# LaurenYTaylor/jsrl-CORL

Hardware: AMD Instinct MI355X
Metric: IQL gradient-steps/sec at batch=256 (D4RL obs/act dims) (higher is better)
Workload: dtype f32; 1 GPU; IQL step on synthetic buffer (obs=17, act=6, 1000000 rows), batch=256 per GPU; global_batch=256, parallelism=single, prepare_rehearsal_steps=1111

## Files before the change

include/iqlhip.h:

```cpp
#ifndef IQLHIP_H
#define IQLHIP_H

#include <stdint.h>

#ifdef __cplusplus
extern "C" {
#endif

#define IQLHIP_VERSION 400
#define IQLHIP_HIDDEN 256
#define IQLHIP_MAX_INPUT 128
#define IQLHIP_MAX_ACTION 32
#define IQLHIP_MAX_WORLD 8
#define IQLHIP_GRAPH_STEPS 64
#define IQLHIP_N_SCORE 8
#define IQLHIP_N_STATS 16

enum {
  IQLHIP_OK = 0,
  IQLHIP_EINVAL = -1,
  IQLHIP_EHIP = -2,
  IQLHIP_ENOTBOUND = -3,
  IQLHIP_EUNSUPPORTED = -4,
  IQLHIP_EINDEX = -5,
  IQLHIP_EEXCHANGE = -6
};

enum { IQLHIP_NET_V = 0, IQLHIP_NET_Q1 = 1, IQLHIP_NET_Q2 = 2, IQLHIP_NET_PI = 3 };
enum { IQLHIP_POLICY_GAUSSIAN = 0, IQLHIP_POLICY_DETERMINISTIC = 1 };

typedef struct {
  int32_t state_dim;
  int32_t action_dim;
  int32_t hidden_dim;
  int32_t n_hidden;
  int32_t policy;
  int32_t max_batch;
} iqlhip_dims;

typedef struct {
  int64_t seg_begin, seg_end;
  int64_t w0, b0, w1, b1, w2, b2, log_std;
  int32_t k_in;
  int32_t d_out;
} iqlhip_net_layout;

typedef struct {
  iqlhip_net_layout net[4];
  int64_t n_params;
  int64_t n_target;
  int64_t target_src;
} iqlhip_layout;

int iqlhip_arena_layout(const iqlhip_dims* dims, iqlhip_layout* out);

typedef struct {
  float iql_tau;
  float beta;
  float discount;
  float tau;
  float one_minus_tau;
  float exp_adv_max;
  float log_std_min, log_std_max;
} iqlhip_hyper;

typedef struct {
  float step_size[3];
  float bc2_sqrt[3];
  float beta2;
  float one_minus_beta1;
  float one_minus_beta2;
  float eps;
  float grad_scale;
  float inv_batch;
} iqlhip_step_scalars;

typedef struct {
  const float* s_dev; const float* a_dev; const float* r_dev; const float* ns_dev; const float* d_dev;
  int64_t ld_s, ld_a, ld_r, ld_ns, ld_d;
  const int64_t* idx_dev;
  int32_t rows;
} iqlhip_batch;

typedef struct iqlhip_ctx iqlhip_ctx;

int iqlhip_version(void);
const char* iqlhip_last_error(void);
// ... 300 lines not shown
```

jsrl-corl_amd/csrc/iqlhip.hip:

```cpp
#include "iqlhip_kernels.h"
#include "iqlhip_lb_kernels.h"
#include "iqlhip_owned.h"

#include <dlfcn.h>

#include <time.h>

#include <algorithm>
#include <cstdarg>
#include <cstdio>
#include <cstdlib>
#include <cstring>
#include <memory>
#include <string>
#include <type_traits>
#include <vector>

#define GRAPH_STEPS IQLHIP_GRAPH_STEPS
static const int kChunkSizes[] = {GRAPH_STEPS, 16, 4, 2, 1};

static thread_local std::string g_err;

static int fail(int code, const char* fmt, ...) {
  char buf[512];
// ... 278 lines not shown
    iqlhip_net_layout& nl = out->net[n];
    nl.k_in = (n == IQLHIP_NET_Q1 || n == IQLHIP_NET_Q2) ? S + A : S;
    nl.d_out = (n == IQLHIP_NET_PI) ? A : 1;
    nl.seg_begin = off;
    nl.w1 = off; off += (int64_t)Hd * Hd;
    nl.w0 = off; off += (int64_t)Hd * nl.k_in;
    nl.b0 = off; off += Hd;
    nl.b1 = off; off += Hd;
    nl.w2 = off; off += (int64_t)nl.d_out * Hd;
    nl.b2 = off; off += up(nl.d_out, 4);
    if (n == IQLHIP_NET_PI && d->policy == IQLHIP_POLICY_GAUSSIAN) { nl.log_std = off; off += up(A, 4); }
    else nl.log_std = -1;
    off = up(off, 64);
    nl.seg_end = off;
  }
  out->n_params = off;
  out->target_src = out->net[IQLHIP_NET_Q1].seg_begin;
  out->n_target = out->net[IQLHIP_NET_Q2].seg_end - out->net[IQLHIP_NET_Q1].seg_begin;
  return IQLHIP_OK;
}

extern "C" int64_t iqlhip_row_stride(int32_t S, int32_t A) { return up(2 * (int64_t)S + A + 2, 4); }

static int xld_host(int k0) { int k0p = (k0 + 3) & ~3; return ((k0p + 29) / 32) * 32 + 2; }

extern "C" int iqlhip_destroy(iqlhip_ctx* c);
extern "C" int iqlhip_xch_shutdown(iqlhip_ctx* c);

static int create_impl(iqlhip_ctx* c, const iqlhip_dims* dims, const iqlhip_hyper* hyper, int device) {
  c->dims = *dims;
  c->hyper = *hyper;
  c->device = device;
  iqlhip_arena_layout(dims, &c->L);
  const int MB = dims->max_batch, A = dims->action_dim;
  c->n_chunk_max = (MB + CHUNK_ROWS - 1) / CHUNK_ROWS;
  c->n_rt_max = (MB + RT_ROWS - 1) / RT_ROWS;
  c->sc.max_batch = MB;
  Owned& own = c->own;
  auto dalloc = [&](float** p, size_t nfloat) { return own.dev(p, nfloat * sizeof(float), 0); };
  HIPCHK(dalloc(&c->sc.h0, (size_t)4 * MB * HID));
  HIPCHK(dalloc(&c->sc.h1, (size_t)4 * MB * HID));
  HIPCHK(dalloc(&c->sc.heads, (size_t)MB * HEAD_LD + (size_t)NSPLIT * MB * A));
  c->row_ld = iqlhip_row_stride(dims->state_dim, A);
  HIPCHK(dalloc(&c->xb, (size_t)MB * c->row_ld));
  HIPCHK(dalloc(&c->xb2, (size_t)MB * c->row_ld));
  HIPCHK(own.pin(&c->losses_host, 4 * sizeof(float)));
  HIPCHK(own.pin(&c->on_row_pin, (size_t)c->row_ld * sizeof(float)));
  HIPCHK(own.pin(&c->on_idx_pin, (size_t)MB * sizeof(long long)));
  HIPCHK(own.pin(&c->on_loss_pin, 4 * sizeof(float)));
  HIPCHK(own.pin(&c->done_pin, 8 * sizeof(unsigned long long), true));
  HIPCHK(own.pin(&c->on_act_pin, (size_t)(IQLHIP_MAX_INPUT + IQLHIP_MAX_ACTION) * sizeof(float)));
  c->act_cap = std::max(MB, IQLHIP_ACT_ROWS);
  HIPCHK(dalloc(&c->xb_act, (size_t)c->act_cap * c->row_ld));
  HIPCHK(dalloc(&c->heads_act, (size_t)c->act_cap * A * NSPLIT));
  HIPCHK(own.dev(&c->drop_bits, (size_t)4 * MB * 8 * sizeof(unsigned), 0xFF));
  HIPCHK(dalloc(&c->sc.slab_a, (size_t)c->n_chunk_max * c->L.n_params));
  size_t sb = 0;
  for (int n = 0; n < 4; ++n) {
    c->sc.slab_b_off[n] = (long long)sb;
    sb += (size_t)c->n_rt_max * ((size_t)HID * c->L.net[n].k_in + HID);
  }
  HIPCHK(dalloc(&c->sc.slab_b, sb));
  HIPCHK(dalloc(&c->sc.loss_parts, 2 * 4 * 64));
  HIPCHK(dalloc(&c->pi_t, (size_t)MB * 65));
  HIPCHK(dalloc(&c->sc.losses, 4));
  HIPCHK(dalloc(&c->flat_tmp, (size_t)c->L.n_params + 4));
  c->k_max = 1024;
  c->ring_cap = c->k_max;
  HIPCHK(own.pin(&c->loss_ring, (size_t)c->ring_cap * 4 * sizeof(float), true));
  HIPCHK(own.dev(&c->sched_cur, (size_t)GRAPH_STEPS * sizeof(iqlhip_step_scalars)));
  HIPCHK(own.dev(&c->sched_call, (size_t)c->k_max * sizeof(iqlhip_step_scalars)));
  for (int i = 0; i < 4; ++i) HIPCHK(own.pin(&c->sched_pin[i], (size_t)c->k_max * sizeof(iqlhip_step_scalars)));
  HIPCHK(own.pin(&c->sched_ack, 8 * sizeof(unsigned long long), true));
  HIPCHK(own.dev(&c->setup_arrivals, 64, 0));
  HIPCHK(own.dev(&c->hdr, HDR_WORDS * sizeof(unsigned long long), 0));
  HIPCHK(own.dev(&c->xstatus, 2 * sizeof(unsigned long long), 0));
  HIPCHK(own.pin(&c->xstatus_host, 2 * sizeof(unsigned long long), true));
  HIPCHK(dalloc(&c->xflat, (size_t)up(c->L.n_params + 4, 64)));
  HIPCHK(hipStreamCreateWithFlags(&c->cap_stream, hipStreamNonBlocking));
#ifdef IQL_STAMPS
  HIPCHK(own.dev(&c->stamps, 4096 * 16 * sizeof(unsigned long long), 0));
#endif
  const int kq = dims->state_dim + dims->action_dim;
  const int ks_ = dims->state_dim;
  const size_t fwd_fixed = (size_t)(RT_ROWS * H0_LD + RT_ROWS * T64_LD + RT_ROWS * (int)c->row_ld +
                                    (((A + 15) & ~15) * W2_LD + 32) + 512 + 16) * sizeof(float);
  auto fits = [&](int k) { return fwd_fixed + (size_t)HID * k * sizeof(float) + 4096 <= (size_t)160 * 1024 - 1024; };
  int w0_lds_k = 0;
  if (kq <= W0_DMA_MAX_K && fits(kq)) w0_lds_k = kq;
  else if (ks_ <= W0_DMA_MAX_K && fits(ks_)) w0_lds_k = ks_;
  if (const char* ov = getenv("IQLHIP_W0_LDS_K")) w0_lds_k = std::min(w0_lds_k, atoi(ov));
  c->w0_lds_k = w0_lds_k;
  if (const char* ov = getenv("IQLHIP_BWD_DONATE_PCT")) c->bwd_donate_pct = std::max(0, std::min(100, atoi(ov)));
  if (const char* ov = getenv("IQLHIP_BWD_SPB_L2")) c->bwd_spb_force = std::max(0, std::min(2, atoi(ov)));
  if (const char* ov = getenv("IQLHIP_FWD_SPB_L2")) c->fwd_spb_force = std::max(0, std::min(2, atoi(ov)));
// ... 480 lines not shown
  const double t = (double)p * 4294967296.0;
  return t >= 4294967295.0 ? 0xFFFFFFFFu : (unsigned)t;
}

static ActDropRec act_drop_record(const iqlhip_ctx* c, int rows) {
  ActDropRec d;
  memset(&d, 0, sizeof d);
  d.active = (c->act_drop_p > 0.f && rows > 0) ? 1 : 0;
  if (!d.active) return d;
  d.bits = c->act_drop_bits;
  d.n_rows = rows;
  d.cap = c->act_cap;
  d.thresh = drop_thresh(c->act_drop_p);
  d.seed = c->act_drop_seed;
  d.call = c->act_drop_calls;
  return d;
}

static void launch_dropmask(const iqlhip_ctx* c, unsigned long long seed, unsigned long long step,
                            const unsigned long long* hdr, int k, hipStream_t st) {
  const int n_words = 2 * c->dims.max_batch * 8;
  hipLaunchKernelGGL(iql_dropmask_kernel, dim3((n_words + 255) / 256), dim3(256), 0, st, c->drop_bits, n_words,
                     drop_thresh(c->drop_p), seed, step, hdr, k);
}

static int upd_blocks(const iqlhip_ctx* c) {
  long long seg_max = 0;
  for (int n = 0; n < 4; ++n) {
    const long long end = (n < 3) ? c->L.net[n + 1].seg_begin : c->L.n_params;
    seg_max = std::max(seg_max, end - c->L.net[n].seg_begin);
  }
  return 8 * (int)((seg_max + 2047) / 2048);
}
struct UpdWords { unsigned s0, s1, s2, s3, end, flags; };
static UpdWords upd_words(const iqlhip_ctx* c, const UpdParams& u) {
  UpdWords w;
  w.s0 = (unsigned)c->L.net[0].seg_begin; w.s1 = (unsigned)c->L.net[1].seg_begin; w.s2 = (unsigned)c->L.net[2].seg_begin;
  w.s3 = (unsigned)c->L.net[3].seg_begin; w.end = (unsigned)c->L.net[3].seg_end;
  w.flags = (u.n_peer == 0 && !u.flat_grads && !u.slab_x && u.n_chunk == 1) ? UPD_EARLY_G : 0u;
  return w;
}
static auto upd_kernel(bool from_table, bool peer, bool lb) {
  return with_bools([](auto NLB, auto NT, auto NP) { return &iql_update_kernel<!NT.value, !NP.value, !NLB.value>; }, !lb, !from_table, !peer);
}
static void launch_upd(const iqlhip_ctx* c, UpdParams u, hipStream_t st, const float* clip = nullptr) {
  const UpdWords w = upd_words(c, u);
  if (clip) {
    if (u.sched) hipLaunchKernelGGL(iql_update_clip_kernel<true>, dim3(upd_blocks(c)), dim3(256), 0, st, u.params, u.m, u.v, u.slab_a,
                                    w.s0, w.s1, w.s2, w.s3, w.end, w.flags, clip, u);
    else hipLaunchKernelGGL(iql_update_clip_kernel<false>, dim3(upd_blocks(c)), dim3(256), 0, st, u.params, u.m, u.v, u.slab_a,
                            w.s0, w.s1, w.s2, w.s3, w.end, w.flags, clip, u);
    return;
  }
  hipLaunchKernelGGL(upd_kernel(u.sched != nullptr, u.n_peer > 0, u.slab_x != nullptr), dim3(upd_blocks(c)),
                     dim3(256), 0, st, u.params, u.m, u.v, u.slab_a, w.s0, w.s1, w.s2, w.s3, w.end, w.flags, u);
}

static void refresh_shadows(const iqlhip_ctx* c, hipStream_t st) {
  if (c->precision != 1) return;
  const long long n = std::max<long long>(c->L.n_params, c->L.n_target);
  hipLaunchKernelGGL(iql_shadow_refresh_kernel, dim3((unsigned)((n / 4 + 255) / 256)), dim3(256), 0, st, c->params, c->target,
                     c->wsh, c->tsh, (long long)c->L.n_params, (long long)c->L.n_target, c->L, c->wimg);
}

static auto flatten_kernel(bool sys, bool lb) {
  return with_bools([](auto NLB, auto NSYS) { return &iql_grad_flatten_kernel<!NSYS.value, !NLB.value>; }, !lb, !sys);
}
static void launch_flatten(const iqlhip_ctx* c, const UpdParams& u, float* out, bool sys, hipStream_t st) {
  const int nb = (int)((c->L.n_params / 4 + 255) / 256);
  hipLaunchKernelGGL(flatten_kernel(sys, u.slab_x != nullptr), dim3(nb), dim3(256), 0, st, u, out);
}

static int read_back(void* dst_host, void* pin, const void* dev, size_t bytes, hipStream_t st, bool sync = true) {
  HIPCHK(hipMemcpyAsync(pin, dev, bytes, hipMemcpyDeviceToHost, st));
  if (!sync) return IQLHIP_OK;
  HIPCHK(hipStreamSynchronize(st));
  if (dst_host) memcpy(dst_host, pin, bytes);
  return IQLHIP_OK;
}

static int stats_parts(const iqlhip_ctx* c) { return upd_blocks(c) / 8 * 2; }
static int ensure_gparts(iqlhip_ctx* c) {
  if (c->stats_part) return IQLHIP_OK;
  c->stats_n_part = stats_parts(c);
  HIPCHK(c->own.dev(&c->stats_part, (size_t)4 * c->stats_n_part * sizeof(float), 0));
  return IQLHIP_OK;
}
extern "C" int iqlhip_set_step_stats(iqlhip_ctx* c, int enabled) {
// ... 1796 lines not shown
static int group_check_call(iqlhip_group* g, const int32_t* rows) {
  if (!g) return fail(IQLHIP_EINVAL, "NULL group");
  int rc = group_check_members(g->m, g->k, g->flags);
  if (rc) return rc;
  for (int i = 0; i < g->k; ++i) {
    if ((rc = group_check_bound(g, i))) return rc;
    if (rows[i] < 1 || rows[i] > g->m[i]->dims.max_batch)
      return fail(IQLHIP_EINVAL, "member %d: batch rows %d outside [1, max_batch=%d]", i, rows[i], g->m[i]->dims.max_batch);
  }
  for (int i = 0; i < g->k; ++i)
    if (g->m[0]->precision == 1 && rows[i] > LB_MIN_ROWS)
      return fail(IQLHIP_EUNSUPPORTED, "bf16 groups take batches of at most %d rows (the large-batch kernels have no group form)", LB_MIN_ROWS);
  for (int i = 0; i < g->k; ++i)
    if ((rc = optional_features_check(g->m[i], rows[i]))) return rc;
  return IQLHIP_OK;
}

static void group_record(iqlhip_group* g, GroupRec& r, int i, const GroupGeom& q, int rows, int n, const float* xb,
                         const iqlhip_step_scalars* sc0, const iqlhip_step_scalars* sched) {
  iqlhip_ctx* c = g->m[i];
  memset(&r, 0, sizeof r);
  r.p = make_step(c, rows, sc0->inv_batch);
  r.p.xb = xb;
  r.p.spb_l2 = q.fwd_l2;
  const BwdWords b = bwd_words(c, r.p, q.n_chunk[i], q.n_rt[i], 0u);
  r.q_heads = b.heads; r.q_xb = b.xb; r.q_h1 = b.h1; r.q_h0 = b.h0; r.q_params = b.params;
  r.q_dims = b.dims; r.q_ldB = b.ldB; r.q_mbc = b.mbc; r.q_rts = b.rts;
  r.u = make_upd(c, sc0, rows, nullptr);
  r.u.sched = sched;
  r.u.sched_idx = 0;
  r.u.loss_ring = g->ring_dev + (size_t)i * IQLHIP_GROUP_MAX_STEPS * 4;
  r.u.ring_slot = 0;
  const UpdWords w = upd_words(c, r.u);
  r.u_p = r.u.params; r.u_m = r.u.m; r.u_v = r.u.v; r.u_slab_a = r.u.slab_a;
  r.u_s0 = w.s0; r.u_s1 = w.s1; r.u_s2 = w.s2; r.u_s3 = w.s3; r.u_end = w.end; r.u_flags = w.flags;
  r.n_steps = n;
  r.xb = (float*)xb;
  r.B = rows;
}

static bool group_draws(const iqlhip_ctx* c) { return c->drop_p > 0.f && !c->drop_inject; }

static GroupDropRec group_drop_record(const iqlhip_ctx* c, int rows) {
  GroupDropRec d;
  memset(&d, 0, sizeof d);
  d.bits = c->drop_bits;
  d.n_rows = rows;
  d.max_batch = c->dims.max_batch;
  d.thresh = drop_thresh(c->drop_p);
  d.active = 1;
  d.seed = c->drop_seed;
  d.step0 = c->drop_step;
  return d;
}

static int group_drop_records_packed(const iqlhip_group* g, GroupDropRec* d, const int32_t* rows) {
  int n = 0;
  if (!(g->flags & IQLHIP_GROUP_DROPOUT)) return 0;
  for (int i = 0; i < g->k; ++i)
    if (group_draws(g->m[i])) d[n++] = group_drop_record(g->m[i], rows[i]);
  return n;
}

static void group_launch_dropmask(iqlhip_group* g, const GroupDropRec* drops, int n_draw, int max_rows, hipStream_t st) {
  if (n_draw == 0) return;
  hipLaunchKernelGGL(iql_dropmask_group_kernel, dim3((2 * max_rows * 8 + 255) / 256, n_draw), dim3(256), 0, st, drops);
  for (int i = 0; i < g->k; ++i)
    if (group_draws(g->m[i])) g->m[i]->drop_step += 1;
// ... 2434 lines not shown
```

jsrl-corl_amd/csrc/iqlhip_kernels.h:

```cpp
#pragma once
#include <hip/hip_runtime.h>
#include <stdint.h>
#include "iqlhip.h"

typedef float f32x4 __attribute__((ext_vector_type(4)));
typedef float f32x2 __attribute__((ext_vector_type(2)));
typedef float f32x4u __attribute__((ext_vector_type(4), aligned(4)));

#define HID 256
#define RT_ROWS 32
#define CHUNK_ROWS 256
#define H0_LD 260
#define H0B_LD 264
#define T64_LD 68
#define NSPLIT 4
#define HEAD_LD 24
#define W0_LDS_MAX_K 64
#define W0_DMA_MAX_K 96
#define W2_LD 68

#define MFMA16(a, b, c) __builtin_amdgcn_mfma_f32_16x16x4f32((a), (b), (c), 0, 0, 0)

typedef __bf16 bf16x8 __attribute__((ext_vector_type(8)));
#define MFMA_BF16(a, b, c) __builtin_amdgcn_mfma_f32_16x16x32_bf16((a), (b), (c), 0, 0, 0)
// ... 824 lines not shown
      const unsigned long long t0 = wall_clock64();
      unsigned long long polls = 0;
      while (__hip_atomic_load(mine, __ATOMIC_RELAXED, __HIP_MEMORY_SCOPE_SYSTEM) < v) {
        __builtin_amdgcn_s_sleep(4);
        if (((++polls) & 63ull) == 0ull && wall_clock64() - t0 > x.timeout_ticks) {
          __hip_atomic_store(x.status, v, __ATOMIC_RELAXED, __HIP_MEMORY_SCOPE_AGENT);
          break;
        }
      }
    }
  }
}

template <bool SYS, bool LB = false>
__global__ __launch_bounds__(256) void iql_grad_flatten_kernel(UpdParams u, float* out) {
  const long long e = ((long long)blockIdx.x * 256 + threadIdx.x) * 4;
  if (e < u.L.n_params) {
    const int net = net_of(u.L, e);
    const f32x4 gv = slab_grad<LB>(u, e, net);
    if (SYS) store16_sys(out + e, gv);
    else *(f32x4*)(out + e) = gv;
  }
  if (blockIdx.x == 0 && threadIdx.x == 0) {
    float s[4];
    loss_words(u, s);
    const float ib = u.sc.inv_batch;
    const f32x4 tail = (f32x4){s[0] * ib, (s[1] * ib + s[2] * ib) * 0.5f, s[3] * ib, 0.f};
    if (SYS) store16_sys(out + u.L.n_params, tail);
    else *(f32x4*)(out + u.L.n_params) = tail;
  }
}

#define UPD_EARLY_G 1u
template <bool FROM_TABLE, bool PEER, bool LB = false>
__global__ __launch_bounds__(256) void iql_update_kernel(float* q_p, float* q_m, float* q_v, const float* q_slab_a, unsigned q_s0,
                                                         unsigned q_s1, unsigned q_s2, unsigned q_s3, unsigned q_end,
                                                         unsigned q_flags, UpdParams u) {
  constexpr int step = 0;
  constexpr bool CLIP = false;
  const float* const q_clip = nullptr;
#include "iqlhip_upd_body.inc"
}
template <bool FROM_TABLE>
__global__ __launch_bounds__(256) void iql_update_clip_kernel(float* q_p, float* q_m, float* q_v, const float* q_slab_a, unsigned q_s0,
                                                              unsigned q_s1, unsigned q_s2, unsigned q_s3, unsigned q_end,
                                                              unsigned q_flags, const float* q_clip, UpdParams u) {
  constexpr int step = 0;
  constexpr bool PEER = false, LB = false, CLIP = true;
#include "iqlhip_upd_body.inc"
}

struct GroupRec {
  StepParams p;
  const float* q_heads; const float* q_xb; const float* q_h1; const float* q_h0; const float* q_params;
  unsigned q_dims, q_ldB, q_mbc, q_rts;
  UpdParams u;
  float* u_p; float* u_m; float* u_v; const float* u_slab_a;
  unsigned u_s0, u_s1, u_s2, u_s3, u_end, u_flags;
  const float* rows;
  long long ld, size;
  unsigned long long seed, offset;
  float* xb;
  int B;
  int n_steps;
  const float* rows_on;
  long long size_on;
  int n_off;
};

template <bool BF16, bool W0DMA, bool MULTI>
__global__ __launch_bounds__(256) __attribute__((amdgpu_waves_per_eu(2))) void iql_fwd_group_kernel(const GroupRec* __restrict__ recs) {
  constexpr bool ONE = false;
  constexpr bool ROW_EXIT = true;
  constexpr bool MIXED_IDLE = false;
  const StepParams& p = recs[blockIdx.y].p;
#include "iqlhip_fwd_body.inc"
}

template <bool BF16, bool FULL>
__global__ __launch_bounds__(256) void iql_bwd_group_kernel(const GroupRec* __restrict__ recs) {
  constexpr bool MULTI = false;
  constexpr bool KPF = false;
  constexpr bool RW = false;
  const float* const rw_w = nullptr;
  float* const rw_td = nullptr;
  const GroupRec& r = recs[blockIdx.y];
  const float* q_heads = r.q_heads; const float* q_xb = r.q_xb; const float* q_h1 = r.q_h1; const float* q_h0 = r.q_h0;
  const float* q_params = r.q_params;
  const unsigned q_dims = r.q_dims, q_ldB = r.q_ldB, q_mbc = r.q_mbc, q_rts = r.q_rts;
  const StepParams& p = r.p;
#include "iqlhip_bwd_body.inc"
}

__global__ __launch_bounds__(256) void iql_update_group_kernel(const GroupRec* __restrict__ recs, int step) {
  constexpr bool FROM_TABLE = true, PEER = false, LB = false;
  const GroupRec& r = recs[blockIdx.y];
  float* q_p = r.u_p; float* q_m = r.u_m; float* q_v = r.u_v; const float* q_slab_a = r.u_slab_a;
  const unsigned q_s0 = r.u_s0, q_s1 = r.u_s1, q_s2 = r.u_s2, q_s3 = r.u_s3, q_end = r.u_end, q_flags = r.u_flags;
  const UpdParams& u = r.u;
  step = min(max(step, 0), r.n_steps - 1);
  constexpr bool CLIP = false;
  const float* const q_clip = nullptr;
#include "iqlhip_upd_body.inc"
}

__global__ __launch_bounds__(256) void iql_gather_group_kernel(const GroupRec* __restrict__ recs, int step) {
  const GroupRec& r = recs[blockIdx.y];
  const int s = min(max(step, 0), r.n_steps - 1);
  gather_rows_drawn(r.rows, r.ld, r.xb, r.B, r.seed, r.offset, (unsigned long long)s * (unsigned long long)r.B,
                    (unsigned long long)r.size, (int)blockIdx.x * 256 + (int)threadIdx.x, (int)gridDim.x * 256);
}

struct GroupDropRec {
  unsigned* bits;
  int n_rows;
  int max_batch;
  unsigned thresh;
  int active;
  unsigned long long seed, step0;
};
__device__ __forceinline__ void group_drop_words(const GroupDropRec& d, unsigned long long step, int first, int stride) {
  const int per = d.n_rows * 8;
  for (int v = first; v < 2 * per; v += stride) {
    const int w = (v < per) ? v : d.max_batch * 8 + (v - per);
    dropmask_words(d.bits, w + 1, d.thresh, d.seed, step, w, w + 1);
  }
}

__global__ __launch_bounds__(256) void iql_dropmask_group_kernel(const GroupDropRec* __restrict__ drops) {
  const GroupDropRec& d = drops[blockIdx.y];
  group_drop_words(d, d.step0, (int)blockIdx.x * 256 + (int)threadIdx.x, (int)gridDim.x * 256);
// ... 155 lines not shown
  if (wave < 3) {
    const int first = (wave == 0) ? 0 : ((wave == 1) ? a.n_part : 3 * a.n_part);
    const int cnt = (wave == 1) ? 2 * a.n_part : a.n_part;
    double acc = 0.0;
    for (int i = lane; i < cnt; i += 64) acc += (double)a.gparts[first + i];
#pragma unroll
    for (int o = 32; o > 0; o >>= 1) acc += __shfl_xor(acc, o);
    if (lane == 0) {
      const float nrm = (float)sqrt(acc);
      const float mx = a.limits[wave];
      float cf = 1.f;
      if (mx < __builtin_inff()) {
        const float q = __fdiv_rn(mx, __fadd_rn(nrm, 1e-6f));
        cf = (q > 1.f) ? 1.f : q;
      }
      a.coef[wave] = cf;
      a.norm[wave] = nrm;
    }
  }
}
__global__ __launch_bounds__(256) void iql_clip_coef_kernel(ClipArgs a) { clip_coef_block(a); }

struct GroupClipRec { ClipArgs a; const float* coef_rd; int enabled; };
__global__ __launch_bounds__(256) void iql_clip_coef_group_kernel(const GroupClipRec* __restrict__ crecs) {
  const GroupClipRec& c = crecs[blockIdx.y];
  if (!c.enabled) return;
  clip_coef_block(c.a);
}
__global__ __launch_bounds__(256) void iql_update_clip_group_kernel(const GroupRec* __restrict__ recs,
                                                                    const GroupClipRec* __restrict__ crecs, int step) {
  constexpr bool FROM_TABLE = true, PEER = false, LB = false, CLIP = true;
  const GroupRec& r = recs[blockIdx.y];
  float* q_p = r.u_p; float* q_m = r.u_m; float* q_v = r.u_v; const float* q_slab_a = r.u_slab_a;
  const unsigned q_s0 = r.u_s0, q_s1 = r.u_s1, q_s2 = r.u_s2, q_s3 = r.u_s3, q_end = r.u_end, q_flags = r.u_flags;
  const float* const q_clip = crecs[blockIdx.y].coef_rd;
  const UpdParams& u = r.u;
  step = min(max(step, 0), r.n_steps - 1);
#include "iqlhip_upd_body.inc"
}

__device__ __forceinline__ void pack_states(float* xb, int ld, int S, int n, const float* s, long long ld_s) {
  const int total = n * ld;
  for (int e = blockIdx.x * blockDim.x + threadIdx.x; e < total; e += gridDim.x * blockDim.x) {
    const int i = e / ld;
    const int c = e - i * ld;
    xb[e] = (c < S) ? s[i * ld_s + c] : 0.f;
  }
}
__global__ void iql_pack_states_kernel(float* xb, int ld, int S, int n, const float* s, long long ld_s) {
  pack_states(xb, ld, S, n, s, ld_s);
}

struct ActDropRec {
  unsigned* bits;
  int n_rows;
  int cap;
  unsigned thresh;
  int active;
  unsigned long long seed, call;
};
__device__ __forceinline__ void act_drop_words(const ActDropRec& d, int first, int stride) {
  const int per = d.n_rows * 8;
  for (int v = first; v < 2 * per; v += stride) {
    const int layer = (v >= per) ? 1 : 0, rq = v - layer * per;
    const uint32_t w = (uint32_t)((rq >> 3) * 16 + layer * 8 + (rq & 7));
    d.bits[layer * d.cap * 8 + rq] = keep_word(w, 0x41445250u , d.thresh, d.seed, d.call);
  }
// ... 488 lines not shown
```

jsrl-corl_amd/csrc/iqlhip_upd_body.inc:

```
  const int ux = (int)(blockIdx.x & 7u), uq = (int)(blockIdx.x >> 3);
  const int net = ux & 3, uhalf = ux >> 2;
  const long long seg_b = (long long)((net == 0) ? q_s0 : ((net == 1) ? q_s1 : ((net == 2) ? q_s2 : q_s3)));
  const long long seg_e = (long long)((net == 0) ? q_s1 : ((net == 1) ? q_s2 : ((net == 2) ? q_s3 : q_end)));
  const long long e = seg_b + (long long)uq * 2048 + (long long)((((int)threadIdx.x >> 4) * 2 + uhalf) * 64 + ((int)threadIdx.x & 15) * 4);
  if (e < seg_e) {
    f32x4 m = *(f32x4*)(q_m + e);
    f32x4 v = *(f32x4*)(q_v + e);
    f32x4 pw = *(f32x4*)(q_p + e);
    const bool early_g = !PEER && !LB && (q_flags & UPD_EARLY_G) != 0u && (e - seg_b) < 65536;
    f32x4 gr = (f32x4){0.f, 0.f, 0.f, 0.f};
    if (early_g) gr = *(const f32x4*)(q_slab_a + e);
    float cf = 1.f;
    if (CLIP) cf = q_clip[(net == IQLHIP_NET_V) ? 0 : ((net == IQLHIP_NET_PI) ? 2 : 1)];
    __builtin_amdgcn_sched_barrier(0);
#define U64(x) ((unsigned long long)(x))
    asm volatile("" ::"s"(U64(u.L.net[0].seg_begin)), "s"(U64(u.L.net[1].seg_begin)), "s"(U64(u.L.net[2].seg_begin)),
                 "s"(U64(u.L.net[3].seg_begin)), "s"(U64(u.L.net[0].w0)), "s"(U64(u.L.net[1].w0)), "s"(U64(u.L.net[2].w0)),
                 "s"(U64(u.L.net[3].w0)), "s"(U64(u.L.net[0].b0)), "s"(U64(u.L.net[1].b0)), "s"(U64(u.L.net[2].b0)),
                 "s"(U64(u.L.net[3].b0)), "s"(u.L.net[0].k_in), "s"(u.L.net[1].k_in), "s"(u.L.net[2].k_in),
                 "s"(u.L.net[3].k_in), "s"(U64(u.slab_b_off[0])), "s"(U64(u.slab_b_off[1])), "s"(U64(u.slab_b_off[2])),
                 "s"(U64(u.slab_b_off[3])), "s"(U64(u.L.n_params)), "s"(U64(u.L.target_src)), "s"(U64((uintptr_t)u.params)),
                 "s"(U64((uintptr_t)u.target)), "s"(U64((uintptr_t)u.m)), "s"(U64((uintptr_t)u.v)),
                 "s"(U64((uintptr_t)u.slab_a)), "s"(U64((uintptr_t)u.slab_b)), "s"(U64((uintptr_t)u.flat_grads)),
                 "s"(U64((uintptr_t)u.sched)));
#undef U64

    const bool is_q = (net == IQLHIP_NET_Q1 || net == IQLHIP_NET_Q2);
    float* tp = u.target + (is_q ? (e - u.L.target_src) : 0);
    f32x4 t = (f32x4){0.f, 0.f, 0.f, 0.f};
    if (is_q) t = *(f32x4*)tp;
    if (PEER) {
      static_assert(IQLHIP_MAX_WORLD == 8, "load16_sys_x8");
      const NetWords nl = net_words(u, net);
      if (u.peer_direct && e >= nl.w0 && e < nl.b0 + HID) {
        const long long stride = (long long)HID * nl.k_in + HID;
        const long long off = nl.slab_b_off + (e - nl.w0);
        gr = (f32x4){0.f, 0.f, 0.f, 0.f};
        for (int r = 0; r < u.n_peer; ++r) {
          f32x4 pv[8];
          const float* pp[8];
#pragma unroll
          for (int j = 0; j < 8; ++j) pp[j] = u.peer_slab_b[r] + off + (long long)min(j, u.n_rt - 1) * stride;
          load16_sys_x8(pv, pp);
          f32x4 gsum = (f32x4){0.f, 0.f, 0.f, 0.f};
#pragma unroll
          for (int j = 0; j < 8; ++j) if (j < u.n_rt) gsum += pv[j];
          gr = (r == 0) ? gsum : gr + gsum;
        }
      } else {
        f32x4 pv[8];
        const float* pp[8];
#pragma unroll
        for (int r = 0; r < 8; ++r) pp[r] = u.peer_flat[min(r, u.n_peer - 1)] + e;
        load16_sys_x8(pv, pp);
        gr = pv[0];
#pragma unroll
        for (int r = 1; r < IQLHIP_MAX_WORLD; ++r) if (r < u.n_peer) gr += pv[r];
      }
    } else if (u.flat_grads) gr = *(const f32x4*)(u.flat_grads + e);
    else if (!early_g) gr = slab_grad<LB>(u, e, net);
    const int grp = (net == IQLHIP_NET_V) ? 0 : ((net == IQLHIP_NET_PI) ? 2 : 1);
    iqlhip_step_scalars sc;
    if (FROM_TABLE) sc = u.sched[u.sched_idx + step];
// ... 74 lines not shown
```

jsrl-corl_amd/iqlhip_binding.py:

```python
from __future__ import annotations

import ctypes as C
import os
from typing import Optional

_HERE = os.path.dirname(os.path.abspath(__file__))
LIB_PATH = os.environ.get("IQLHIP_LIB", os.path.join(_HERE, "libiqlhip.so"))

IQLHIP_HIDDEN = 256
IQLHIP_ACT_ROWS = 4096
IQLHIP_MAX_WORLD = 8
IQLHIP_GRAPH_STEPS = 64
IQLHIP_N_STATS = 16
STAT_NAMES = ("v_mean", "next_v_mean", "q1_mean", "q2_mean", "target_q_mean", "td_target_mean", "q_gap_mean",
              "adv_mean", "adv_min", "adv_max", "adv_pos_frac", "exp_adv_mean", "exp_adv_clamped_frac",
              "grad_norm_vf", "grad_norm_qf", "grad_norm_actor")
IQLHIP_N_SCORE = 8
SCORE_NAMES = ("v", "next_v", "q1", "q2", "target_q", "adv", "exp_adv", "bc")
SPREAD_NAMES = tuple("mean_" + name for name in SCORE_NAMES) + tuple("std_" + name for name in SCORE_NAMES)
IQLHIP_MAX_GROUP = 16
IQLHIP_GROUP_ACT_WAIT = 1
IQLHIP_GROUP_DROPOUT = 1
IQLHIP_GROUP_MAX_STEPS = 1024
IQLHIP_GROUP_TS_CONTINUE = 1
# ... 25 lines not shown
    _fields_ = [("net", NetLayout * 4), ("n_params", C.c_int64), ("n_target", C.c_int64),
                ("target_src", C.c_int64)]


class Hyper(C.Structure):
    _fields_ = [("iql_tau", C.c_float), ("beta", C.c_float), ("discount", C.c_float), ("tau", C.c_float),
                ("one_minus_tau", C.c_float), ("exp_adv_max", C.c_float), ("log_std_min", C.c_float),
                ("log_std_max", C.c_float)]


class StepScalars(C.Structure):
    _fields_ = [("step_size", C.c_float * 3), ("bc2_sqrt", C.c_float * 3), ("beta2", C.c_float),
                ("one_minus_beta1", C.c_float), ("one_minus_beta2", C.c_float), ("eps", C.c_float),
                ("grad_scale", C.c_float), ("inv_batch", C.c_float)]


class VarScalars(C.Structure):
    _fields_ = [("step_size", C.c_float), ("bc2_sqrt", C.c_float), ("beta2", C.c_float), ("one_minus_beta1", C.c_float),
                ("one_minus_beta2", C.c_float), ("eps", C.c_float), ("aligned_rewards", C.c_int32), ("reserved", C.c_int32)]


class Batch(C.Structure):
    _fields_ = [("s_dev", C.c_void_p), ("a_dev", C.c_void_p), ("r_dev", C.c_void_p), ("ns_dev", C.c_void_p),
                ("d_dev", C.c_void_p),
                ("ld_s", C.c_int64), ("ld_a", C.c_int64), ("ld_r", C.c_int64), ("ld_ns", C.c_int64),
                ("ld_d", C.c_int64),
                ("idx_dev", C.c_void_p), ("rows", C.c_int32)]


SYMBOLS = [
    ("iqlhip_version", C.c_int, []),
    ("iqlhip_last_error", C.c_char_p, []),
    ("iqlhip_arena_layout", C.c_int, [C.POINTER(Dims), C.POINTER(Layout)]),
    ("iqlhip_create", C.c_int, [C.POINTER(Dims), C.POINTER(Hyper), C.c_int, C.POINTER(C.c_void_p)]),
    ("iqlhip_destroy", C.c_int, [C.c_void_p]),
    ("iqlhip_set_hyper", C.c_int, [C.c_void_p, C.POINTER(Hyper)]),
    ("iqlhip_bind", C.c_int, [C.c_void_p, C.c_void_p, C.c_void_p, C.c_void_p, C.c_void_p]),
    ("iqlhip_set_precision", C.c_int, [C.c_void_p, C.c_int]),
    ("iqlhip_set_dropout", C.c_int, [C.c_void_p, C.c_float, C.c_uint64]),
    ("iqlhip_set_act_dropout", C.c_int, [C.c_void_p, C.c_float, C.c_uint64]),
    ("iqlhip_get_act_dropout_counter", C.c_int, [C.c_void_p, C.POINTER(C.c_uint64)]),
    ("iqlhip_set_act_dropout_counter", C.c_int, [C.c_void_p, C.c_uint64]),
    ("iqlhip_get_counters", C.c_int, [C.c_void_p, C.POINTER(C.c_uint64)]),
    ("iqlhip_set_counters", C.c_int, [C.c_void_p, C.POINTER(C.c_uint64)]),
    ("iqlhip_debug_write_masks", C.c_int, [C.c_void_p, C.c_void_p, C.c_void_p, C.c_int32, C.c_void_p]),
    ("iqlhip_step", C.c_int, [C.c_void_p, C.POINTER(Batch), C.POINTER(StepScalars), C.c_void_p]),
    ("iqlhip_step_rw", C.c_int, [C.c_void_p, C.POINTER(Batch), C.POINTER(StepScalars), C.c_void_p, C.c_void_p, C.c_void_p]),
    ("iqlhip_forward_backward_rw", C.c_int, [C.c_void_p, C.POINTER(Batch), C.POINTER(StepScalars), C.c_void_p, C.c_void_p,
                                             C.c_void_p, C.c_void_p]),
    ("iqlhip_draw_indices_weighted_is", C.c_int, [C.c_void_p, C.c_void_p, C.c_int64, C.c_void_p, C.c_uint64, C.c_uint64,
                                                  C.c_int64, C.c_float, C.c_void_p]),
    ("iqlhip_step_sync", C.c_int, [C.c_void_p, C.POINTER(Batch), C.POINTER(StepScalars), C.POINTER(C.c_float), C.c_void_p]),
    ("iqlhip_step_begin", C.c_int, [C.c_void_p, C.POINTER(Batch), C.POINTER(StepScalars), C.c_void_p]),
    ("iqlhip_step_wait", C.c_int, [C.c_void_p, C.POINTER(C.c_float), C.c_void_p]),
    ("iqlhip_online_step", C.c_int, [C.c_void_p, C.c_void_p, C.c_int64, C.c_int64, C.c_int64, C.c_void_p, C.c_void_p,
                                     C.c_int32, C.POINTER(StepScalars), C.POINTER(C.c_float), C.c_void_p, C.c_float,
                                     C.c_uint64, C.c_void_p, C.c_void_p]),
    ("iqlhip_online_step_mixed", C.c_int, [C.c_void_p, C.c_void_p, C.c_int64, C.c_int64, C.c_int64, C.c_void_p, C.c_void_p,
                                           C.c_int32, C.POINTER(StepScalars), C.POINTER(C.c_float), C.c_void_p, C.c_float,
                                           C.c_uint64, C.c_void_p, C.c_void_p, C.c_void_p, C.c_int64, C.c_void_p,
                                           C.c_int32]),
    ("iqlhip_train_steps_mixed", C.c_int, [C.c_void_p, C.c_void_p, C.c_int64, C.c_void_p, C.c_int64, C.c_int64, C.c_int32,
                                           C.c_int32, C.c_void_p, C.c_int32, C.c_uint64, C.c_uint64, C.c_void_p]),
    ("iqlhip_train_steps_mixed_prepare", C.c_int, [C.c_void_p, C.c_void_p, C.c_void_p, C.c_int64, C.c_int32, C.c_int32,
                                                   C.c_float, C.c_void_p]),
    ("iqlhip_forward_backward", C.c_int, [C.c_void_p, C.POINTER(Batch), C.POINTER(StepScalars), C.c_void_p, C.c_void_p]),
# ... 236 lines not shown
```

Before: 52110 steps/s.

## Hoist target and slab_b gradient loads ahead of update kernel scalar setup

Packs the segment bounds and dims into fewer kernel arguments and places slab_b directly after slab_a in one allocation, so the update kernel can address the per-row-tile gradient partials from q_slab_a at a fixed offset. Target weights and the slab_b partial sums (up to 8 tiles) are then loaded early, before the scheduling barrier and the scalar-argument block, instead of afterwards. The aim is to overlap these global loads with the m/v/p loads in the fused Adam update. In exchange, host-side validation becomes more complex, the kernel issues extra speculative loads, and register pressure rises from holding 8 f32x4 values.

```diff
diff --git a/include/iqlhip.h b/include/iqlhip.h
--- a/include/iqlhip.h
+++ b/include/iqlhip.h
@@ -53,6 +53,7 @@
 } iqlhip_layout;
 
 int iqlhip_arena_layout(const iqlhip_dims* dims, iqlhip_layout* out);
+int iqlhip_upd_pack_bounds(const iqlhip_layout* layout, int32_t state_dim, int32_t action_dim, uint32_t out[3]);
 
 typedef struct {
   float iql_tau;
diff --git a/jsrl-corl_amd/csrc/iqlhip.hip b/jsrl-corl_amd/csrc/iqlhip.hip
--- a/jsrl-corl_amd/csrc/iqlhip.hip
+++ b/jsrl-corl_amd/csrc/iqlhip.hip
@@ -334,6 +334,10 @@
   c->hyper = *hyper;
   c->device = device;
   iqlhip_arena_layout(dims, &c->L);
+  {
+    uint32_t pk[3];
+    if (int rc = iqlhip_upd_pack_bounds(&c->L, dims->state_dim, dims->action_dim, pk)) return rc;
+  }
   const int MB = dims->max_batch, A = dims->action_dim;
   c->n_chunk_max = (MB + CHUNK_ROWS - 1) / CHUNK_ROWS;
   c->n_rt_max = (MB + RT_ROWS - 1) / RT_ROWS;
@@ -356,13 +360,14 @@
   HIPCHK(dalloc(&c->xb_act, (size_t)c->act_cap * c->row_ld));
   HIPCHK(dalloc(&c->heads_act, (size_t)c->act_cap * A * NSPLIT));
   HIPCHK(own.dev(&c->drop_bits, (size_t)4 * MB * 8 * sizeof(unsigned), 0xFF));
-  HIPCHK(dalloc(&c->sc.slab_a, (size_t)c->n_chunk_max * c->L.n_params));
   size_t sb = 0;
   for (int n = 0; n < 4; ++n) {
     c->sc.slab_b_off[n] = (long long)sb;
     sb += (size_t)c->n_rt_max * ((size_t)HID * c->L.net[n].k_in + HID);
   }
-  HIPCHK(dalloc(&c->sc.slab_b, sb));
+  const size_t sa = (size_t)c->n_chunk_max * c->L.n_params;
+  HIPCHK(dalloc(&c->sc.slab_a, sa + sb));
+  c->sc.slab_b = c->sc.slab_a + sa;
   HIPCHK(dalloc(&c->sc.loss_parts, 2 * 4 * 64));
   HIPCHK(dalloc(&c->pi_t, (size_t)MB * 65));
   HIPCHK(dalloc(&c->sc.losses, 4));
@@ -909,12 +914,56 @@
   }
   return 8 * (int)((seg_max + 2047) / 2048);
 }
-struct UpdWords { unsigned s0, s1, s2, s3, end, flags; };
+struct UpdWords { const float* t; unsigned b0, b1, b2, sb; };
+extern "C" int iqlhip_upd_pack_bounds(const iqlhip_layout* L, int32_t state_dim, int32_t action_dim, uint32_t out[3]) {
+  if (!L || !out) return fail(IQLHIP_EINVAL, "NULL argument");
+  unsigned units[5];
+  for (int n = 0; n < 5; ++n) {
+    const int64_t b = (n < 4) ? L->net[n].seg_begin : L->net[3].seg_end;
+    if (b < 0 || (b & 63) != 0 || (b >> 6) > (int64_t)UPD_PACK_MAX_UNITS)
+      return fail(IQLHIP_EUNSUPPORTED, "segment bound %lld is not a multiple of 64 below %u * 64", (long long)b, UPD_PACK_MAX_UNITS + 1u);
+    if (n > 0 && n < 4 && L->net[n - 1].seg_end != b) return fail(IQLHIP_EUNSUPPORTED, "segments are not contiguous");
+    units[n] = (unsigned)(b >> 6);
+  }
+  if (units[0] != 0u) return fail(IQLHIP_EUNSUPPORTED, "the first segment does not begin at 0");
+  if (state_dim < 1 || state_dim > 127 || action_dim < 1 || action_dim > 63)
+    return fail(IQLHIP_EUNSUPPORTED, "dims outside the packed fields (state_dim < 128, action_dim < 64)");
+  out[0] = units[1] | (units[2] << 16);
+  out[1] = units[3] | (units[4] << 16);
+  out[2] = ((unsigned)state_dim << 16) | ((unsigned)action_dim << 23);
+  return IQLHIP_OK;
+}
 static UpdWords upd_words(const iqlhip_ctx* c, const UpdParams& u) {
   UpdWords w;
-  w.s0 = (unsigned)c->L.net[0].seg_begin; w.s1 = (unsigned)c->L.net[1].seg_begin; w.s2 = (unsigned)c->L.net[2].seg_begin;
-  w.s3 = (unsigned)c->L.net[3].seg_begin; w.end = (unsigned)c->L.net[3].seg_end;
-  w.flags = (u.n_peer == 0 && !u.flat_grads && !u.slab_x && u.n_chunk == 1) ? UPD_EARLY_G : 0u;
+  uint32_t pk[3] = {0u, 0u, 0u};
+  (void)iqlhip_upd_pack_bounds(&c->L, c->dims.state_dim, c->dims.action_dim, pk);
+  w.b0 = pk[0]; w.b1 = pk[1]; w.b2 = pk[2]; w.sb = 0u;
+  const iqlhip_layout& L = c->L;
+  const int S = c->dims.state_dim, A = c->dims.action_dim;
+  unsigned flags = 0u;
+  const bool plain = u.n_peer == 0 && !u.flat_grads && !u.slab_x;
+  if (plain && u.n_chunk == 1) flags |= UPD_EARLY_G;
+  bool t_ok = plain && u.target && L.target_src == L.net[IQLHIP_NET_Q1].seg_begin &&
+              L.net[IQLHIP_NET_Q2].seg_begin == L.net[IQLHIP_NET_Q1].seg_end &&
+              L.n_target == L.net[IQLHIP_NET_Q2].seg_end - L.net[IQLHIP_NET_Q1].seg_begin;
+  w.t = t_ok ? (const float*)((uintptr_t)u.target - (uintptr_t)L.target_src * sizeof(float)) : nullptr;
+  if (t_ok) flags |= UPD_EARLY_T;
+  bool k_ok = true;
+  for (int n = 0; n < 4; ++n) {
+    const bool q = (n == IQLHIP_NET_Q1 || n == IQLHIP_NET_Q2);
+    k_ok = k_ok && L.net[n].k_in == (q ? S + A : S) && L.net[n].w0 == L.net[n].seg_begin + 65536 &&
+           L.net[n].b0 == L.net[n].w0 + (long long)HID * L.net[n].k_in;
+  }
+  const long long sV = (long long)HID * S + HID, sQ = (long long)HID * (S + A) + HID;
+  const long long rt_max = u.slab_b_off[1] / sV;
+  const long long d = (u.slab_a && u.slab_b) ? (long long)(u.slab_b - u.slab_a) : -1;
+  if ((flags & UPD_EARLY_G) && k_ok && u.n_rt >= 1 && u.n_rt <= 8 && rt_max >= u.n_rt && rt_max <= 512 && u.slab_b_off[0] == 0 &&
+      u.slab_b_off[1] == rt_max * sV && u.slab_b_off[2] == rt_max * (sV + sQ) && u.slab_b_off[3] == rt_max * (sV + 2 * sQ) &&
+      d > 0 && (d & 63) == 0 && (d >> 6) < (1ll << 19)) {
+    flags |= UPD_EARLY_SB;
+    w.sb = (unsigned)(d >> 6) | ((unsigned)(rt_max - 1) << 19) | ((unsigned)(u.n_rt - 1) << 28);
+  }
+  w.b2 |= flags;
   return w;
 }
 static auto upd_kernel(bool from_table, bool peer, bool lb) {
@@ -924,13 +973,13 @@
   const UpdWords w = upd_words(c, u);
   if (clip) {
     if (u.sched) hipLaunchKernelGGL(iql_update_clip_kernel<true>, dim3(upd_blocks(c)), dim3(256), 0, st, u.params, u.m, u.v, u.slab_a,
-                                    w.s0, w.s1, w.s2, w.s3, w.end, w.flags, clip, u);
+                                    w.t, w.b0, w.b1, w.b2, w.sb, clip, u);
     else hipLaunchKernelGGL(iql_update_clip_kernel<false>, dim3(upd_blocks(c)), dim3(256), 0, st, u.params, u.m, u.v, u.slab_a,
-                            w.s0, w.s1, w.s2, w.s3, w.end, w.flags, clip, u);
+                            w.t, w.b0, w.b1, w.b2, w.sb, clip, u);
     return;
   }
   hipLaunchKernelGGL(upd_kernel(u.sched != nullptr, u.n_peer > 0, u.slab_x != nullptr), dim3(upd_blocks(c)),
-                     dim3(256), 0, st, u.params, u.m, u.v, u.slab_a, w.s0, w.s1, w.s2, w.s3, w.end, w.flags, u);
+                     dim3(256), 0, st, u.params, u.m, u.v, u.slab_a, w.t, w.b0, w.b1, w.b2, w.sb, u);
 }
 
 static void refresh_shadows(const iqlhip_ctx* c, hipStream_t st) {
@@ -2793,8 +2842,8 @@
   r.u.loss_ring = g->ring_dev + (size_t)i * IQLHIP_GROUP_MAX_STEPS * 4;
   r.u.ring_slot = 0;
   const UpdWords w = upd_words(c, r.u);
-  r.u_p = r.u.params; r.u_m = r.u.m; r.u_v = r.u.v; r.u_slab_a = r.u.slab_a;
-  r.u_s0 = w.s0; r.u_s1 = w.s1; r.u_s2 = w.s2; r.u_s3 = w.s3; r.u_end = w.end; r.u_flags = w.flags;
+  r.u_p = r.u.params; r.u_m = r.u.m; r.u_v = r.u.v; r.u_slab_a = r.u.slab_a; r.u_t = w.t;
+  r.u_b0 = w.b0; r.u_b1 = w.b1; r.u_b2 = w.b2; r.u_sb = w.sb;
   r.n_steps = n;
   r.xb = (float*)xb;
   r.B = rows;
diff --git a/jsrl-corl_amd/csrc/iqlhip_kernels.h b/jsrl-corl_amd/csrc/iqlhip_kernels.h
--- a/jsrl-corl_amd/csrc/iqlhip_kernels.h
+++ b/jsrl-corl_amd/csrc/iqlhip_kernels.h
@@ -880,19 +880,25 @@
 }
 
 #define UPD_EARLY_G 1u
+#define UPD_EARLY_T 2u
+#define UPD_EARLY_SB 4u
+#define UPD_PACK_MAX_UNITS 65535u
+static_assert(4u * (65536u + 256u * IQLHIP_MAX_INPUT + 256u * (IQLHIP_MAX_ACTION + 3u) + 128u) / 64u <= UPD_PACK_MAX_UNITS,
+              "segment bounds in units of 64 floats must fit 16 bits");
+static_assert(IQLHIP_MAX_INPUT <= 128 && IQLHIP_MAX_ACTION < 64, "S in 7 bits, A in 6 bits of q_b2");
 template <bool FROM_TABLE, bool PEER, bool LB = false>
-__global__ __launch_bounds__(256) void iql_update_kernel(float* q_p, float* q_m, float* q_v, const float* q_slab_a, unsigned q_s0,
-                                                         unsigned q_s1, unsigned q_s2, unsigned q_s3, unsigned q_end,
-                                                         unsigned q_flags, UpdParams u) {
+__global__ __launch_bounds__(256) void iql_update_kernel(float* q_p, float* q_m, float* q_v, const float* q_slab_a, const float* q_t,
+                                                         unsigned q_b0, unsigned q_b1, unsigned q_b2, unsigned q_sb,
+                                                         UpdParams u) {
   constexpr int step = 0;
   constexpr bool CLIP = false;
   const float* const q_clip = nullptr;
 #include "iqlhip_upd_body.inc"
 }
 template <bool FROM_TABLE>
-__global__ __launch_bounds__(256) void iql_update_clip_kernel(float* q_p, float* q_m, float* q_v, const float* q_slab_a, unsigned q_s0,
-                                                              unsigned q_s1, unsigned q_s2, unsigned q_s3, unsigned q_end,
-                                                              unsigned q_flags, const float* q_clip, UpdParams u) {
+__global__ __launch_bounds__(256) void iql_update_clip_kernel(float* q_p, float* q_m, float* q_v, const float* q_slab_a, const float* q_t,
+                                                              unsigned q_b0, unsigned q_b1, unsigned q_b2, unsigned q_sb,
+                                                              const float* q_clip, UpdParams u) {
   constexpr int step = 0;
   constexpr bool PEER = false, LB = false, CLIP = true;
 #include "iqlhip_upd_body.inc"
@@ -903,8 +909,8 @@
   const float* q_heads; const float* q_xb; const float* q_h1; const float* q_h0; const float* q_params;
   unsigned q_dims, q_ldB, q_mbc, q_rts;
   UpdParams u;
-  float* u_p; float* u_m; float* u_v; const float* u_slab_a;
-  unsigned u_s0, u_s1, u_s2, u_s3, u_end, u_flags;
+  float* u_p; float* u_m; float* u_v; const float* u_slab_a; const float* u_t;
+  unsigned u_b0, u_b1, u_b2, u_sb;
   const float* rows;
   long long ld, size;
   unsigned long long seed, offset;
@@ -944,7 +950,8 @@
   constexpr bool FROM_TABLE = true, PEER = false, LB = false;
   const GroupRec& r = recs[blockIdx.y];
   float* q_p = r.u_p; float* q_m = r.u_m; float* q_v = r.u_v; const float* q_slab_a = r.u_slab_a;
-  const unsigned q_s0 = r.u_s0, q_s1 = r.u_s1, q_s2 = r.u_s2, q_s3 = r.u_s3, q_end = r.u_end, q_flags = r.u_flags;
+  const float* q_t = r.u_t;
+  const unsigned q_b0 = r.u_b0, q_b1 = r.u_b1, q_b2 = r.u_b2, q_sb = r.u_sb;
   const UpdParams& u = r.u;
   step = min(max(step, 0), r.n_steps - 1);
   constexpr bool CLIP = false;
@@ -1166,7 +1173,8 @@
   constexpr bool FROM_TABLE = true, PEER = false, LB = false, CLIP = true;
   const GroupRec& r = recs[blockIdx.y];
   float* q_p = r.u_p; float* q_m = r.u_m; float* q_v = r.u_v; const float* q_slab_a = r.u_slab_a;
-  const unsigned q_s0 = r.u_s0, q_s1 = r.u_s1, q_s2 = r.u_s2, q_s3 = r.u_s3, q_end = r.u_end, q_flags = r.u_flags;
+  const float* q_t = r.u_t;
+  const unsigned q_b0 = r.u_b0, q_b1 = r.u_b1, q_b2 = r.u_b2, q_sb = r.u_sb;
   const float* const q_clip = crecs[blockIdx.y].coef_rd;
   const UpdParams& u = r.u;
   step = min(max(step, 0), r.n_steps - 1);
diff --git a/jsrl-corl_amd/csrc/iqlhip_upd_body.inc b/jsrl-corl_amd/csrc/iqlhip_upd_body.inc
--- a/jsrl-corl_amd/csrc/iqlhip_upd_body.inc
+++ b/jsrl-corl_amd/csrc/iqlhip_upd_body.inc
@@ -1,34 +1,61 @@
   const int ux = (int)(blockIdx.x & 7u), uq = (int)(blockIdx.x >> 3);
   const int net = ux & 3, uhalf = ux >> 2;
-  const long long seg_b = (long long)((net == 0) ? q_s0 : ((net == 1) ? q_s1 : ((net == 2) ? q_s2 : q_s3)));
+  const unsigned q_s1 = (q_b0 & 0xFFFFu) << 6, q_s2 = (q_b0 >> 16) << 6, q_s3 = (q_b1 & 0xFFFFu) << 6, q_end = (q_b1 >> 16) << 6;
+  const unsigned q_flags = q_b2 & 0xFFFFu;
+  const long long seg_b = (long long)((net == 0) ? 0u : ((net == 1) ? q_s1 : ((net == 2) ? q_s2 : q_s3)));
   const long long seg_e = (long long)((net == 0) ? q_s1 : ((net == 1) ? q_s2 : ((net == 2) ? q_s3 : q_end)));
   const long long e = seg_b + (long long)uq * 2048 + (long long)((((int)threadIdx.x >> 4) * 2 + uhalf) * 64 + ((int)threadIdx.x & 15) * 4);
+  const bool is_q = (net == IQLHIP_NET_Q1 || net == IQLHIP_NET_Q2);
   if (e < seg_e) {
     f32x4 m = *(f32x4*)(q_m + e);
     f32x4 v = *(f32x4*)(q_v + e);
     f32x4 pw = *(f32x4*)(q_p + e);
-    const bool early_g = !PEER && !LB && (q_flags & UPD_EARLY_G) != 0u && (e - seg_b) < 65536;
+    const bool early_t = !PEER && !LB && is_q && (q_flags & UPD_EARLY_T) != 0u;
+    f32x4 t = (f32x4){0.f, 0.f, 0.f, 0.f};
+    if (early_t) t = *(const f32x4*)(q_t + e);
+    const bool early_a = !PEER && !LB && (q_flags & UPD_EARLY_G) != 0u;
+    const bool early_b = early_a && (q_flags & UPD_EARLY_SB) != 0u && uq >= 32;
+    const bool early_g = early_a && (uq < 32 || early_b);
     f32x4 gr = (f32x4){0.f, 0.f, 0.f, 0.f};
     if (early_g) gr = *(const f32x4*)(q_slab_a + e);
+    f32x4 sv[8];
+    bool in_b = false;
+    const int e_nrt = (int)(q_sb >> 28) + 1;
+    if (early_b) {
+      const int dS = (int)((q_b2 >> 16) & 127u), dA = (int)((q_b2 >> 23) & 63u);
+      const int k_in = is_q ? dS + dA : dS;
+      const long long w0 = seg_b + 65536;
+      const unsigned stride = (unsigned)(HID * k_in + HID);
+      in_b = e >= w0 && e < w0 + stride;
+      const unsigned rt_max = ((q_sb >> 19) & 511u) + 1u;
+      const unsigned sV = (unsigned)(HID * dS + HID), sQ = (unsigned)(HID * (dS + dA) + HID);
+      const unsigned noff = rt_max * ((net == 0) ? 0u : ((net == 1) ? sV : ((net == 2) ? sV + sQ : sV + 2u * sQ)));
+      const float* base = q_slab_a + (size_t)(((q_sb & 0x7FFFFu) << 6) + noff + (in_b ? (unsigned)(e - w0) : 0u));
+#pragma unroll
+      for (int j = 0; j < 8; ++j) sv[j] = *(const f32x4*)(base + (size_t)((unsigned)min(j, e_nrt - 1) * stride));
+    }
     float cf = 1.f;
     if (CLIP) cf = q_clip[(net == IQLHIP_NET_V) ? 0 : ((net == IQLHIP_NET_PI) ? 2 : 1)];
     __builtin_amdgcn_sched_barrier(0);
 #define U64(x) ((unsigned long long)(x))
-    asm volatile("" ::"s"(U64(u.L.net[0].seg_begin)), "s"(U64(u.L.net[1].seg_begin)), "s"(U64(u.L.net[2].seg_begin)),
-                 "s"(U64(u.L.net[3].seg_begin)), "s"(U64(u.L.net[0].w0)), "s"(U64(u.L.net[1].w0)), "s"(U64(u.L.net[2].w0)),
+    asm volatile("" ::"s"(U64(u.L.net[0].w0)), "s"(U64(u.L.net[1].w0)), "s"(U64(u.L.net[2].w0)),
                  "s"(U64(u.L.net[3].w0)), "s"(U64(u.L.net[0].b0)), "s"(U64(u.L.net[1].b0)), "s"(U64(u.L.net[2].b0)),
                  "s"(U64(u.L.net[3].b0)), "s"(u.L.net[0].k_in), "s"(u.L.net[1].k_in), "s"(u.L.net[2].k_in),
                  "s"(u.L.net[3].k_in), "s"(U64(u.slab_b_off[0])), "s"(U64(u.slab_b_off[1])), "s"(U64(u.slab_b_off[2])),
-                 "s"(U64(u.slab_b_off[3])), "s"(U64(u.L.n_params)), "s"(U64(u.L.target_src)), "s"(U64((uintptr_t)u.params)),
-                 "s"(U64((uintptr_t)u.target)), "s"(U64((uintptr_t)u.m)), "s"(U64((uintptr_t)u.v)),
-                 "s"(U64((uintptr_t)u.slab_a)), "s"(U64((uintptr_t)u.slab_b)), "s"(U64((uintptr_t)u.flat_grads)),
-                 "s"(U64((uintptr_t)u.sched)));
+                 "s"(U64(u.slab_b_off[3])), "s"(U64(u.L.n_params)), "s"(U64(u.L.target_src)),
+                 "s"(U64((uintptr_t)u.target)), "s"(U64((uintptr_t)u.slab_a)), "s"(U64((uintptr_t)u.slab_b)),
+                 "s"(U64((uintptr_t)u.flat_grads)), "s"(U64((uintptr_t)u.sched)));
 #undef U64
 
-    const bool is_q = (net == IQLHIP_NET_Q1 || net == IQLHIP_NET_Q2);
-    float* tp = u.target + (is_q ? (e - u.L.target_src) : 0);
-    f32x4 t = (f32x4){0.f, 0.f, 0.f, 0.f};
-    if (is_q) t = *(f32x4*)tp;
+    if (early_b) {
+      f32x4 gsum = (f32x4){0.f, 0.f, 0.f, 0.f};
+#pragma unroll
+      for (int j = 0; j < 8; ++j) if (j < e_nrt) gsum += sv[j];
+      if (e_nrt == 1) gsum = sv[0];
+      gr = in_b ? gsum : gr;
+    }
+    float* tp = early_t ? (float*)q_t + e : u.target + (is_q ? (e - u.L.target_src) : 0);
+    if (is_q && !early_t) t = *(f32x4*)tp;
     if (PEER) {
       static_assert(IQLHIP_MAX_WORLD == 8, "load16_sys_x8");
       const NetWords nl = net_words(u, net);
diff --git a/jsrl-corl_amd/iqlhip_binding.py b/jsrl-corl_amd/iqlhip_binding.py
--- a/jsrl-corl_amd/iqlhip_binding.py
+++ b/jsrl-corl_amd/iqlhip_binding.py
@@ -81,6 +81,7 @@
     ("iqlhip_version", C.c_int, []),
     ("iqlhip_last_error", C.c_char_p, []),
     ("iqlhip_arena_layout", C.c_int, [C.POINTER(Dims), C.POINTER(Layout)]),
+    ("iqlhip_upd_pack_bounds", C.c_int, [C.POINTER(Layout), C.c_int32, C.c_int32, C.POINTER(C.c_uint32)]),
     ("iqlhip_create", C.c_int, [C.POINTER(Dims), C.POINTER(Hyper), C.c_int, C.POINTER(C.c_void_p)]),
     ("iqlhip_destroy", C.c_int, [C.c_void_p]),
     ("iqlhip_set_hyper", C.c_int, [C.c_void_p, C.POINTER(Hyper)]),
```

Measured after the change: 52090 steps/s. About the same (-0.0%).
